# anoma/taiga

Measured on NVIDIA H100. Metric: partial-tx proofs/sec, higher is better.
Workload: dtype u32x8 (255-bit Montgomery integers, Pasta Fp/Fq)

## Files before the change

### taiga_b200/csrc/msm_batch.cu

```cuda
#define TB_NOINLINE_MUL 0
#include <cuda.h>
#include <algorithm>
#include <memory>
#include <type_traits>
#include "common.cuh"
#include "kernels.cuh"

namespace tb {

constexpr int BA_THREADS = 256;
constexpr int BA_M = 32;
constexpr int BA_BWD_MINB = 3;
constexpr int BA_MAX_NB = 4096;
constexpr int SORT_THREADS = 1024;
constexpr int SORT_TILE = 1024;
constexpr int SORT_BOX = 256;

__device__ __forceinline__ void block_scan_excl(uint32_t* v, int n, uint32_t* tmp) {
  const int T = blockDim.x, t = threadIdx.x, per = (n + T - 1) / T;
  const int b0 = t * per, b1 = min(n, b0 + per);
  uint32_t local = 0;
  for (int i = b0; i < b1; ++i) local += v[i];
  uint32_t incl = local;
  const int lane = t & 31, warp = t >> 5, nw = (T + 31) >> 5;
#pragma unroll
  for (int d = 1; d < 32; d <<= 1) { uint32_t o = __shfl_up_sync(0xffffffffu, incl, d); if (lane >= d) incl += o; }
  if (lane == 31) tmp[warp] = incl;
  __syncthreads();
  if (warp == 0) {
    uint32_t w = lane < nw ? tmp[lane] : 0u, wi = w;
#pragma unroll
    for (int d = 1; d < 32; d <<= 1) { uint32_t o = __shfl_up_sync(0xffffffffu, wi, d); if (lane >= d) wi += o; }
    if (lane < nw) tmp[lane] = wi - w;
    if (lane == nw - 1) v[n] = wi;
  }
  __syncthreads();
  uint32_t run = tmp[warp] + incl - local;
  for (int i = b0; i < b1; ++i) { uint32_t x = v[i]; v[i] = run; run += x; }
  __syncthreads();
}

__device__ __forceinline__ uint32_t smem_u32(const void* p) { return (uint32_t)__cvta_generic_to_shared(p); }
__device__ __forceinline__ void mbar_init(uint64_t* bar, uint32_t count) {
  asm volatile("mbarrier.init.shared::cta.b64 [%0], %1;" ::"r"(smem_u32(bar)), "r"(count) : "memory");
}
__device__ __forceinline__ void mbar_expect_tx(uint64_t* bar, uint32_t bytes) {
  asm volatile("mbarrier.arrive.expect_tx.shared::cta.b64 _, [%0], %1;" ::"r"(smem_u32(bar)), "r"(bytes) : "memory");
}
__device__ __forceinline__ void mbar_wait(uint64_t* bar, uint32_t parity) {
  uint32_t done = 0;
  for (uint32_t spin = 0; spin < (1u << 26); ++spin) {
    asm volatile("{ .reg .pred p; mbarrier.try_wait.parity.shared::cta.b64 p, [%1], %2; selp.u32 %0, 1, 0, p; }" : "=r"(done) : "r"(smem_u32(bar)), "r"(parity) : "memory");
    if (done) return;
  }
  __trap();
}
__device__ __forceinline__ void tma_load_tile(void* dst, const CUtensorMap* map, uint64_t* bar, int scalar0, int item) {
  asm volatile("cp.async.bulk.tensor.3d.shared::cluster.global.tile.mbarrier::complete_tx::bytes [%0], [%1, {%3, %4, %5}], [%2];"
               ::"r"(smem_u32(dst)), "l"(map), "r"(smem_u32(bar)), "r"(0), "r"(scalar0), "r"(item) : "memory");
}

template <class S, int CT>
__global__ void __launch_bounds__(SORT_THREADS) msm_sort_kernel(const __grid_constant__ CUtensorMap smap, const S* __restrict__ extras, int N, int n_extra, int c_rt, int W_rt,
                                                                 int NB, int table_stride, uint32_t* __restrict__ counts, uint32_t* __restrict__ entries, long long cap0,
                                                                 unsigned long long* __restrict__ total_entries) {
  const int c = CT ? CT : c_rt, W = CT ? (256 + CT - 1) / CT : W_rt;
  extern __shared__ __align__(128) uint8_t sort_smem[];
  S* tile = reinterpret_cast<S*>(sort_smem);
  uint64_t* bars = reinterpret_cast<uint64_t*>(sort_smem + 2 * SORT_TILE * sizeof(S));
  uint32_t* hist = reinterpret_cast<uint32_t*>(bars + 2);
  uint32_t* tmp = hist + NB + 1;
  const int k = blockIdx.x, t = threadIdx.x;
  const uint32_t half = 1u << (c - 1);
  const int ntiles = (N + SORT_TILE - 1) / SORT_TILE;
  if (t == 0) { mbar_init(&bars[0], 1); mbar_init(&bars[1], 1); asm volatile("fence.mbarrier_init.release.cluster;" ::: "memory"); }
  for (int b = t; b <= NB; b += SORT_THREADS) hist[b] = 0;
  __syncthreads();
  uint32_t* ent = entries + (long long)k * cap0;

  auto digits = [&](const S& sm, uint32_t idx, auto scatter_c) {
    constexpr bool scatter = decltype(scatter_c)::value;
    S s = sm.from_mont();
    if (s.is_zero()) return;
    uint32_t carry = 0;
#pragma unroll
    for (int w = 0; w < W; ++w) {
      const int bit = w * c, limb = bit >> 5, off = bit & 31;
      uint64_t v64 = s.l[limb];
      if (limb + 1 < 8) v64 |= (uint64_t)s.l[limb + 1] << 32;
      uint32_t v = ((uint32_t)(v64 >> off) & ((1u << c) - 1)) + carry, neg = 0;
      if (v > half) { v = (1u << c) - v; neg = 1; carry = 1; } else carry = 0;
      if (v) {
        if (scatter) { const uint32_t pos = atomicAdd(&hist[v - 1], 1u); ent[pos] = (uint32_t)(w * table_stride + idx) | (neg << 31); }
        else atomicAdd(&hist[v - 1], 1u);
      }
    }
  };
  auto issue = [&](int stage, int it) {
    const int s0 = it * SORT_TILE;
    int nbox = (N - s0 + SORT_BOX - 1) / SORT_BOX; if (nbox > SORT_TILE / SORT_BOX) nbox = SORT_TILE / SORT_BOX;
    mbar_expect_tx(&bars[stage], (uint32_t)(nbox * SORT_BOX * sizeof(S)));
    for (int j = 0; j < nbox; ++j) tma_load_tile(tile + stage * SORT_TILE + j * SORT_BOX, &smap, &bars[stage], s0 + j * SORT_BOX, k);
  };
  uint32_t phase[2] = {0, 0};
  for (int pass = 0; pass < 2; ++pass) {
    if (t == 0) issue(0, 0);
    for (int it = 0; it < ntiles; ++it) {
      const int st = it & 1;
      if (t == 0 && it + 1 < ntiles) issue(st ^ 1, it + 1);
      mbar_wait(&bars[st], phase[st]); phase[st] ^= 1;
      const int i = it * SORT_TILE + t;
      if (i < N) { if (pass) digits(tile[st * SORT_TILE + t], (uint32_t)i, std::true_type()); else digits(tile[st * SORT_TILE + t], (uint32_t)i, std::false_type()); }
      __syncthreads();
    }
    if (t < n_extra) { const S ex = ldg_fe(extras + (long long)k * n_extra + t); if (pass) digits(ex, (uint32_t)(N + t), std::true_type()); else digits(ex, (uint32_t)(N + t), std::false_type()); }
    __syncthreads();
    if (pass == 0) {
      for (int b = t; b < NB; b += SORT_THREADS) counts[(long long)k * NB + b] = hist[b];
      __syncthreads();
      block_scan_excl(hist, NB, tmp);
      if (t == 0) atomicAdd(total_entries, (unsigned long long)hist[NB]);
    }
  }
}

template <class F> __device__ __forceinline__ void sts_fe(uint4* lo, uint4* hi, int idx, const F& v) {
  lo[idx] = make_uint4(v.l[0], v.l[1], v.l[2], v.l[3]); hi[idx] = make_uint4(v.l[4], v.l[5], v.l[6], v.l[7]);
}
template <class F> __device__ __forceinline__ F lds_fe(const uint4* lo, const uint4* hi, int idx) {
  uint4 x = lo[idx], y = hi[idx]; F v;
  v.l[0] = x.x; v.l[1] = x.y; v.l[2] = x.z; v.l[3] = x.w; v.l[4] = y.x; v.l[5] = y.y; v.l[6] = y.z; v.l[7] = y.w; return v;
}

enum { PK_ADD = 0, PK_DBL, PK_COPY1, PK_COPY2, PK_INF };
constexpr int META_KIND_SHIFT = 28;
constexpr uint32_t META_IN0_MASK = (1u << META_KIND_SHIFT) - 1;

struct RoundOffsets {
  uint32_t* off_cur; uint32_t* off_nxt; uint32_t n_next;
  __device__ __forceinline__ void build(uint8_t* smem, const uint32_t* __restrict__ counts0, int NB, int round) {
    off_cur = reinterpret_cast<uint32_t*>(smem); off_nxt = off_cur + (NB + 4);
    uint32_t* tmp = off_nxt + (NB + 4);
    for (int b = threadIdx.x; b < NB; b += blockDim.x) {
      const uint32_t c0 = counts0[b], cr = (c0 + ((1u << round) - 1)) >> round;
      off_cur[b] = cr; off_nxt[b] = (cr + 1) >> 1;
    }
    __syncthreads();
    block_scan_excl(off_cur, NB, tmp);
    block_scan_excl(off_nxt, NB, tmp);
    n_next = off_nxt[NB];
  }
  __device__ __forceinline__ void locate(uint32_t q, int NB, uint32_t& in0, bool& two, int& hint) const {
    int lo = hint;
#pragma unroll 1
    for (int s = 0; s < 6 && off_nxt[lo + 1] <= q; ++s) ++lo;
    if (off_nxt[lo + 1] <= q) {
      int hi = NB;
      while (hi - lo > 1) { const int mid = (lo + hi) >> 1; if (off_nxt[mid] <= q) lo = mid; else hi = mid; }
    }
    hint = lo;
    in0 = off_cur[lo] + 2 * (q - off_nxt[lo]);
    two = in0 + 1 < off_cur[lo + 1];
  }
};
constexpr size_t ba_off_bytes(int NB) { return (size_t)(2 * (NB + 4) + 32) * 4; }

template <class B> struct Planes {
  B* x; long long cap;
  __device__ __forceinline__ B ldx(uint32_t pos) const { return ldg_fe(x + pos); }
  __device__ __forceinline__ Aff<B> ld(uint32_t pos) const { Aff<B> p; p.x = ldg_fe(x + pos); p.y = ldg_fe(x + cap + pos); return p; }
  __device__ __forceinline__ void st(uint32_t pos, const Aff<B>& p) const { st_fe(x + pos, p.x); st_fe(x + cap + pos, p.y); }
};
template <class B> __device__ __forceinline__ Aff<B> table_point(const Aff<B>* table, uint32_t e) {
  Aff<B> p = ldg_aff(table + (e & 0x7fffffffu));
  if (e >> 31) p.y = p.y.neg();
  return p;
}
template <class B> __device__ __forceinline__ int classify_pair(const Aff<B>& p1, const Aff<B>& p2, B& den) {
  if (p2.is_inf()) return PK_COPY1;
  if (p1.is_inf()) return PK_COPY2;
  den = p2.x - p1.x;
  if (!den.is_zero()) return PK_ADD;
  if (p1.y == p2.y && !p1.y.is_zero()) { den = p1.y.dbl(); return PK_DBL; }
  return PK_INF;
}

__global__ void __launch_bounds__(BA_THREADS) msm_ba_count_kernel(const uint32_t* __restrict__ counts0, int NB, int R, uint32_t* __restrict__ n_items) {
  __shared__ uint32_t red[BA_THREADS / 32];
  const int k = blockIdx.x, t = threadIdx.x;
  for (int r = 0; r <= R; ++r) {
    uint32_t s = 0;
    for (int b = t; b < NB; b += BA_THREADS) s += (counts0[(long long)k * NB + b] + ((1u << r) - 1)) >> r;
    for (int d = 16; d >= 1; d >>= 1) s += __shfl_down_sync(0xffffffffu, s, d);
    if ((t & 31) == 0) red[t >> 5] = s;
    __syncthreads();
    if (t == 0) { uint32_t tot = 0; for (int w = 0; w < BA_THREADS / 32; ++w) tot += red[w]; n_items[(long long)k * (R + 1) + r] = tot; }
    __syncthreads();
  }
}

template <class B, bool FIRST>
__global__ void __launch_bounds__(BA_THREADS) msm_ba_fwd_kernel(const uint32_t* __restrict__ counts0, int NB, int round, const uint32_t* __restrict__ entries,
                                                                 const Aff<B>* __restrict__ table, const B* __restrict__ items_in, long long cap_in, long long cap_out,
                                                                 B* __restrict__ pre, B* __restrict__ tree, uint32_t* __restrict__ meta, uint2* __restrict__ eidx,
                                                                 const uint32_t* __restrict__ n_items, int R) {
  extern __shared__ __align__(16) uint8_t ba_smem[];
  const int k = blockIdx.y, t = threadIdx.x;
  const uint32_t Q0 = blockIdx.x * (BA_M * BA_THREADS);
  if (Q0 >= n_items[(long long)k * (R + 1) + round + 1]) return;
  RoundOffsets ro; ro.build(ba_smem, counts0 + (long long)k * NB, NB, round);
  const uint32_t* ent_k = entries + (long long)k * cap_in;
  const Planes<B> in{const_cast<B*>(items_in) + 2 * (long long)k * cap_in, cap_in};
  B* pre_k = pre + 2 * (long long)k * cap_out;
  uint32_t* meta_k = meta + (long long)k * cap_out;
  uint2* eidx_k = eidx + (long long)k * cap_out;
  B acc = B::one();
  int hint = 0;
#pragma unroll 1
  for (int i = 0; i < BA_M; ++i) {
    const uint32_t q = Q0 + (uint32_t)i * BA_THREADS + t;
    if (q >= ro.n_next) break;
    uint32_t in0; bool two; ro.locate(q, NB, in0, two, hint);
    st_fe(pre_k + q, acc);
    int kind = PK_COPY1;
    uint2 e = make_uint2(0, 0);
    if (FIRST) { e.x = __ldg(ent_k + in0); if (two) e.y = __ldg(ent_k + in0 + 1); eidx_k[q] = e; }
    if (two) {
      const B x1 = FIRST ? ldg_fe(&table[e.x & 0x7fffffffu].x) : in.ldx(in0), x2 = FIRST ? ldg_fe(&table[e.y & 0x7fffffffu].x) : in.ldx(in0 + 1);
      B den = x2 - x1;
      kind = PK_ADD;
      if (den.is_zero() || x1.is_zero() || x2.is_zero()) {
        const Aff<B> p1 = FIRST ? table_point(table, e.x) : in.ld(in0), p2 = FIRST ? table_point(table, e.y) : in.ld(in0 + 1);
        kind = classify_pair(p1, p2, den);
      }
      if (kind == PK_ADD || kind == PK_DBL) acc = acc * den;
    }
    meta_k[q] = in0 | (uint32_t)kind << META_KIND_SHIFT;
  }
  __syncthreads();
  B* nd = reinterpret_cast<B*>(ba_smem);
  nd[BA_THREADS + t] = acc;
  __syncthreads();
  for (int w = BA_THREADS >> 1; w >= 1; w >>= 1) {
    if (t < w) nd[w + t] = nd[2 * (w + t)] * nd[2 * (w + t) + 1];
    __syncthreads();
  }
  B* tr = tree + ((long long)k * gridDim.x + blockIdx.x) * (2 * BA_THREADS);
  st_fe(tr + t, t ? nd[t] : B::one()); st_fe(tr + BA_THREADS + t, nd[BA_THREADS + t]);
}

template <class B>
__global__ void msm_ba_inv_kernel(B* __restrict__ tree, uint32_t n_trees) {
  const uint32_t i = blockIdx.x * blockDim.x + threadIdx.x;
  if (i >= n_trees) return;
  B* root = tree + (size_t)i * (2 * BA_THREADS) + 1;
  st_fe(root, ld_fe(root).inv());
}

template <class B, bool FIRST>
__global__ void __launch_bounds__(BA_THREADS, BA_BWD_MINB) msm_ba_bwd_kernel(const Aff<B>* __restrict__ table, const B* __restrict__ items_in, long long cap_in,
                                                                 B* __restrict__ items_out, long long cap_out, const B* __restrict__ tree,
                                                                 const uint32_t* __restrict__ meta, const uint2* __restrict__ eidx, const uint32_t* __restrict__ n_items, int round, int R) {
  extern __shared__ __align__(16) uint8_t ba_smem[];
  const int k = blockIdx.y, t = threadIdx.x;
  const uint32_t Q0 = blockIdx.x * (BA_M * BA_THREADS);
  const uint32_t n_next = n_items[(long long)k * (R + 1) + round + 1];
  if (Q0 >= n_next) return;
  B* nd = reinterpret_cast<B*>(ba_smem);
  { const B* tr = tree + ((long long)k * gridDim.x + blockIdx.x) * (2 * BA_THREADS);
    nd[t] = ld_fe(tr + t); nd[BA_THREADS + t] = ld_fe(tr + BA_THREADS + t); }
  __syncthreads();
  for (int w = 1; w < BA_THREADS; w <<= 1) {
    B child_inv;
    const int node = w + (t >> 1);
    if (t < 2 * w) child_inv = nd[node] * nd[2 * node + ((t & 1) ^ 1)];
    __syncthreads();
    if (t < 2 * w) nd[2 * node + (t & 1)] = child_inv;
    __syncthreads();
  }
  B inv_run = nd[BA_THREADS + t];
  const Planes<B> in{const_cast<B*>(items_in) + 2 * (long long)k * cap_in, cap_in}, out{items_out + 2 * (long long)k * cap_out, cap_out};
  const uint32_t* meta_k = meta + (long long)k * cap_out;
  const uint2* eidx_k = eidx + (long long)k * cap_out;
  const B* pre_k = out.x + cap_out;
  int last = BA_M - 1;
  while (last >= 0 && Q0 + (uint32_t)last * BA_THREADS + t >= n_next) --last;
#pragma unroll 1
  for (int i = last; i >= 0; --i) {
    const uint32_t q = Q0 + (uint32_t)i * BA_THREADS + t;
    const uint32_t mt = __ldg(meta_k + q);
    const uint2 e = FIRST ? __ldg(eidx_k + q) : make_uint2(0, 0);
    const uint32_t in0 = mt & META_IN0_MASK, kind = mt >> META_KIND_SHIFT;
    const Aff<B> p1 = FIRST ? table_point(table, e.x) : in.ld(in0);
    Aff<B> r;
    if (kind <= PK_DBL) {
      Aff<B> p2 = p1;
      B num, den;
      if (kind == PK_ADD) { p2 = FIRST ? table_point(table, e.y) : in.ld(in0 + 1); num = p2.y - p1.y; den = p2.x - p1.x; }
      else { const B x2 = p1.x.sqr(); num = x2.dbl() + x2; den = p1.y.dbl(); }
      const B dinv = inv_run * ld_fe(pre_k + q);
      inv_run = inv_run * den;
      const B lam = num * dinv;
      r.x = lam.sqr() - p1.x - p2.x;
      r.y = lam * (p1.x - r.x) - p1.y;
    } else {
      r = p1;
      if (kind == PK_COPY2) r = FIRST ? table_point(table, e.y) : in.ld(in0 + 1);
      else if (kind == PK_INF) r = Aff<B>::inf();
    }
    out.st(q, r);
  }
}

template <class B>
__global__ void __launch_bounds__(BA_THREADS) msm_ba_finish_kernel(const uint32_t* __restrict__ counts0, int NB, int round, const B* __restrict__ items, long long cap,
                                                                    Xyzz<B>* __restrict__ buckets) {
  extern __shared__ __align__(16) uint8_t fin_smem[];
  uint32_t* off = reinterpret_cast<uint32_t*>(fin_smem);
  uint32_t* tmp = off + NB + 4;
  const int k = blockIdx.y, t = threadIdx.x;
  for (int b = t; b < NB; b += BA_THREADS) { uint32_t c0 = counts0[(long long)k * NB + b]; off[b] = (c0 + ((1u << round) - 1)) >> round; }
  __syncthreads();
  block_scan_excl(off, NB, tmp);
  const int b = blockIdx.x * BA_THREADS + t;
  if (b >= NB) return;
  Xyzz<B> acc = Xyzz<B>::inf();
  const Planes<B> it{const_cast<B*>(items) + 2 * (long long)k * cap, cap};
  for (uint32_t p = off[b]; p < off[b + 1]; ++p) acc.add_affine(it.ld(p));
  buckets[(long long)k * NB + b] = acc;
}

typedef CUresult (*EncodeTiledFn)(CUtensorMap*, CUtensorMapDataType, cuuint32_t, void*, const cuuint64_t*, const cuuint64_t*, const cuuint32_t*, const cuuint32_t*,
                                  CUtensorMapInterleave, CUtensorMapSwizzle, CUtensorMapL2promotion, CUtensorMapFloatOOBfill);
static EncodeTiledFn encode_tiled_fn() {
  static EncodeTiledFn fn = nullptr;
  if (!fn) {
    void* p = nullptr; cudaDriverEntryPointQueryResult qr;
    TB_CUDA(cudaGetDriverEntryPoint("cuTensorMapEncodeTiled", &p, cudaEnableDefault, &qr));
    if (qr != cudaDriverEntryPointSuccess || !p) throw CudaError("cuTensorMapEncodeTiled is not available from this driver");
    fn = reinterpret_cast<EncodeTiledFn>(p);
  }
  return fn;
}

template <class B, bool FIRST>
static void launch_round(Ctx* ctx, dim3 grid, size_t fwd_smem, size_t bwd_smem, const uint32_t* counts, int NB, int r, const uint32_t* entries, const Aff<B>* table, const B* in,
                         long long cap_in, B* out, long long cap_out, B* pre, B* tree, uint32_t* meta, uint2* eidx, const uint32_t* n_items, int R, uint32_t n_trees) {
  ctx->opt_in_smem(msm_ba_fwd_kernel<B, FIRST>, fwd_smem);
  ctx->opt_in_smem(msm_ba_bwd_kernel<B, FIRST>, bwd_smem);
  launch(ctx, msm_ba_fwd_kernel<B, FIRST>, grid, BA_THREADS, fwd_smem, counts, NB, r, entries, table, in, cap_in, cap_out, pre, tree, meta, eidx, n_items, R);
  launch(ctx, msm_ba_inv_kernel<B>, (n_trees + 63) / 64, 64, 0, tree, n_trees);
  launch(ctx, msm_ba_bwd_kernel<B, FIRST>, grid, BA_THREADS, bwd_smem, table, in, cap_in, out, cap_out, tree, meta, eidx, n_items, r, R);
}

bool msm_batch_applicable(int N, int K, const MsmConfig& cfg, int c) {
  if (cfg.table_windows <= 0 || (1 << (c - 1)) > BA_MAX_NB || c < 6) return false;
  const long long min_terms = tb_tune("TB_MSM_BA_MIN_TERMS", 1 << 21);
  return (long long)N * K >= min_terms;
}

template <class B, class S>
void msm_batch_buckets(Ctx* ctx, const S* scalars, long long sstride, const Aff<B>* table, int N, int K, int c, int W, int table_stride, const S* extras, int n_extra,
                       Xyzz<B>* buckets) {
  const int NB = 1 << (c - 1);
  TB_REQUIRE(((uintptr_t)scalars & 15) == 0 && (sstride * (long long)sizeof(S)) % 16 == 0, "scalar vectors must be 16-byte aligned for TMA");
  const long long cap0 = (long long)(N + n_extra) * W;
  std::vector<long long> cap(1, cap0);
  const int R = tb_tune("TB_MSM_BA_ROUNDS", 10);
  TB_REQUIRE(R >= 1 && R <= 20, "TB_MSM_BA_ROUNDS out of range");
  for (int r = 0; r < R; ++r) cap.push_back((cap.back() + NB + 1) / 2);
  TB_REQUIRE(cap0 <= (long long)META_IN0_MASK + 1, "too many MSM entries for the pair index of meta");
  const int Kc_max = tb_tune("TB_MSM_BA_CHUNK", ctx->sm_count);
  const int Kc = K < Kc_max ? K : Kc_max;
  DevBuf<uint32_t> counts(ctx, (size_t)Kc * NB), entries(ctx, (size_t)Kc * cap0);
  const size_t eidx_fe = ((size_t)Kc * cap[1] + 3) / 4;
  DevBuf<B> itA(ctx, (size_t)Kc * 2 * cap[1]), itB(ctx, std::max(R > 1 ? (size_t)(Kc * 2 * cap[2]) : (size_t)0, eidx_fe));
  uint2* eidx = reinterpret_cast<uint2*>(itB.get());
  const size_t sort_smem = 2 * SORT_TILE * sizeof(S) + 16 + (size_t)(NB + 1 + 32) * 4 + 16;
  const size_t fwd_smem = std::max(ba_off_bytes(NB), (size_t)2 * BA_THREADS * sizeof(B));
  const size_t bwd_smem = (size_t)2 * BA_THREADS * sizeof(B);
  const size_t fin_smem = (size_t)(NB + 4 + 32) * 4;
  ctx->opt_in_smem(msm_sort_kernel<S, 13>, sort_smem);
  ctx->opt_in_smem(msm_sort_kernel<S, 0>, sort_smem);
  ctx->opt_in_smem(msm_ba_finish_kernel<B>, fin_smem);
  const long long pairs_per_cta = (long long)BA_M * BA_THREADS;
  const unsigned ctas1 = (unsigned)((cap[1] + pairs_per_cta - 1) / pairs_per_cta);
  DevBuf<B> tree(ctx, (size_t)Kc * ctas1 * 2 * BA_THREADS);
  DevBuf<uint32_t> meta(ctx, (size_t)Kc * cap[1]), n_items(ctx, (size_t)Kc * (R + 1));
  for (int k0 = 0; k0 < K; k0 += Kc) {
    const int kc = K - k0 < Kc ? K - k0 : Kc;
    { ProfScope ps(ctx, PC_MSM_SORT);
      CUtensorMap smap;
      const cuuint64_t dims[3] = {8, (cuuint64_t)N, (cuuint64_t)kc};
      const cuuint64_t strides[2] = {sizeof(S), (cuuint64_t)sstride * sizeof(S)};
      const cuuint32_t box[3] = {8, SORT_BOX, 1}, estr[3] = {1, 1, 1};
      CUresult cr = encode_tiled_fn()(&smap, CU_TENSOR_MAP_DATA_TYPE_UINT32, 3, const_cast<S*>(scalars + (long long)k0 * sstride), dims, strides, box, estr,
                                      CU_TENSOR_MAP_INTERLEAVE_NONE, CU_TENSOR_MAP_SWIZZLE_NONE, CU_TENSOR_MAP_L2_PROMOTION_L2_128B, CU_TENSOR_MAP_FLOAT_OOB_FILL_NONE);
      if (cr != CUDA_SUCCESS) throw CudaError("cuTensorMapEncodeTiled failed for the scalar tensor (" + std::to_string((int)cr) + ")");
      const S* ex = extras ? extras + (long long)k0 * n_extra : nullptr;
      if (c == 13) launch(ctx, msm_sort_kernel<S, 13>, kc, SORT_THREADS, sort_smem, smap, ex, N, extras ? n_extra : 0, c, W, NB, table_stride, counts.get(), entries.get(), cap0, ctx->d_msm_adds.get());
      else launch(ctx, msm_sort_kernel<S, 0>, kc, SORT_THREADS, sort_smem, smap, ex, N, extras ? n_extra : 0, c, W, NB, table_stride, counts.get(), entries.get(), cap0, ctx->d_msm_adds.get()); }
    { ProfScope ps(ctx, PC_MSM_ACCUM);
      launch(ctx, msm_ba_count_kernel, kc, BA_THREADS, 0, counts.get(), NB, R, n_items.get());
      for (int r = 0; r < R; ++r) {
        const B* in = (r & 1) ? itA.get() : itB.get();
        B* out = (r & 1) ? itB.get() : itA.get();
        const unsigned gx = (unsigned)((cap[r + 1] + pairs_per_cta - 1) / pairs_per_cta);
        dim3 grid(gx, kc);
        const uint32_t n_trees = gx * (uint32_t)kc;
        (r == 0 ? launch_round<B, true> : launch_round<B, false>)(ctx, grid, fwd_smem, bwd_smem, counts.get(), NB, r, entries.get(), table, in, r == 0 ? cap0 : cap[r], out,
                                                                  cap[r + 1], out + cap[r + 1], tree.get(), meta.get(), eidx, n_items.get(), R, n_trees);
      }
      const B* last = (R & 1) ? itA.get() : itB.get();
      launch(ctx, msm_ba_finish_kernel<B>, dim3((NB + BA_THREADS - 1) / BA_THREADS, kc), BA_THREADS, fin_smem, counts.get(), NB, R, last, cap[R], buckets + (size_t)k0 * NB); }
  }
}

template void msm_batch_buckets<Fq, Fp>(Ctx*, const Fp*, long long, const Aff<Fq>*, int, int, int, int, int, const Fp*, int, Xyzz<Fq>*);
template void msm_batch_buckets<Fp, Fq>(Ctx*, const Fq*, long long, const Aff<Fp>*, int, int, int, int, int, const Fq*, int, Xyzz<Fp>*);

}
```

Baseline: 18.34.

## Group batch-affine reduction rounds per thread and fuse next-round forward into backward pass

```diff
diff --git a/taiga_b200/csrc/msm_batch.cu b/taiga_b200/csrc/msm_batch.cu
--- a/taiga_b200/csrc/msm_batch.cu
+++ b/taiga_b200/csrc/msm_batch.cu
@@ -9,8 +9,9 @@
 namespace tb {
 
 constexpr int BA_THREADS = 256;
-constexpr int BA_M = 32;
-constexpr int BA_BWD_MINB = 3;
+constexpr int BA_ITEMS = 64;
+constexpr int BA_GROUP = 4;
+constexpr int BA_BWD_MINB = 2;
 constexpr int BA_MAX_NB = 4096;
 constexpr int SORT_THREADS = 1024;
 constexpr int SORT_TILE = 1024;
@@ -133,42 +134,12 @@
 }
 
 enum { PK_ADD = 0, PK_DBL, PK_COPY1, PK_COPY2, PK_INF };
-constexpr int META_KIND_SHIFT = 28;
-constexpr uint32_t META_IN0_MASK = (1u << META_KIND_SHIFT) - 1;
-
-struct RoundOffsets {
-  uint32_t* off_cur; uint32_t* off_nxt; uint32_t n_next;
-  __device__ __forceinline__ void build(uint8_t* smem, const uint32_t* __restrict__ counts0, int NB, int round) {
-    off_cur = reinterpret_cast<uint32_t*>(smem); off_nxt = off_cur + (NB + 4);
-    uint32_t* tmp = off_nxt + (NB + 4);
-    for (int b = threadIdx.x; b < NB; b += blockDim.x) {
-      const uint32_t c0 = counts0[b], cr = (c0 + ((1u << round) - 1)) >> round;
-      off_cur[b] = cr; off_nxt[b] = (cr + 1) >> 1;
-    }
-    __syncthreads();
-    block_scan_excl(off_cur, NB, tmp);
-    block_scan_excl(off_nxt, NB, tmp);
-    n_next = off_nxt[NB];
-  }
-  __device__ __forceinline__ void locate(uint32_t q, int NB, uint32_t& in0, bool& two, int& hint) const {
-    int lo = hint;
-#pragma unroll 1
-    for (int s = 0; s < 6 && off_nxt[lo + 1] <= q; ++s) ++lo;
-    if (off_nxt[lo + 1] <= q) {
-      int hi = NB;
-      while (hi - lo > 1) { const int mid = (lo + hi) >> 1; if (off_nxt[mid] <= q) lo = mid; else hi = mid; }
-    }
-    hint = lo;
-    in0 = off_cur[lo] + 2 * (q - off_nxt[lo]);
-    two = in0 + 1 < off_cur[lo + 1];
-  }
-};
-constexpr size_t ba_off_bytes(int NB) { return (size_t)(2 * (NB + 4) + 32) * 4; }
 
 template <class B> struct Planes {
   B* x; long long cap;
   __device__ __forceinline__ B ldx(uint32_t pos) const { return ldg_fe(x + pos); }
   __device__ __forceinline__ Aff<B> ld(uint32_t pos) const { Aff<B> p; p.x = ldg_fe(x + pos); p.y = ldg_fe(x + cap + pos); return p; }
+  __device__ __forceinline__ Aff<B> ld_own(uint32_t pos) const { Aff<B> p; p.x = ld_fe(x + pos); p.y = ld_fe(x + cap + pos); return p; }
   __device__ __forceinline__ void st(uint32_t pos, const Aff<B>& p) const { st_fe(x + pos, p.x); st_fe(x + cap + pos, p.y); }
 };
 template <class B> __device__ __forceinline__ Aff<B> table_point(const Aff<B>* table, uint32_t e) {
@@ -185,57 +156,78 @@
   return PK_INF;
 }
 
-__global__ void __launch_bounds__(BA_THREADS) msm_ba_count_kernel(const uint32_t* __restrict__ counts0, int NB, int R, uint32_t* __restrict__ n_items) {
-  __shared__ uint32_t red[BA_THREADS / 32];
+__global__ void __launch_bounds__(BA_THREADS) msm_ba_count_kernel(const uint32_t* __restrict__ counts0, int NB, int R, int S, uint32_t* __restrict__ offs,
+                                                                   uint32_t* __restrict__ blks) {
+  extern __shared__ __align__(16) uint32_t cnt_smem[];
+  uint32_t* v = cnt_smem; uint32_t* tmp = v + NB + 1;
   const int k = blockIdx.x, t = threadIdx.x;
   for (int r = 0; r <= R; ++r) {
-    uint32_t s = 0;
-    for (int b = t; b < NB; b += BA_THREADS) s += (counts0[(long long)k * NB + b] + ((1u << r) - 1)) >> r;
-    for (int d = 16; d >= 1; d >>= 1) s += __shfl_down_sync(0xffffffffu, s, d);
-    if ((t & 31) == 0) red[t >> 5] = s;
-    __syncthreads();
-    if (t == 0) { uint32_t tot = 0; for (int w = 0; w < BA_THREADS / 32; ++w) tot += red[w]; n_items[(long long)k * (R + 1) + r] = tot; }
-    __syncthreads();
-  }
-}
+    for (int pass = 0; pass < (r < R ? 2 : 1); ++pass) {
+      const int g = min(S, R - r);
+      for (int b = t; b < NB; b += BA_THREADS) {
+        const uint32_t a = (counts0[(long long)k * NB + b] + ((1u << r) - 1)) >> r;
+        v[b] = pass ? (a + ((1u << g) - 1)) >> g : a;
+      }
+      __syncthreads();
+      block_scan_excl(v, NB, tmp);
+      uint32_t* dst = pass ? blks + ((long long)k * R + r) * (NB + 1) : offs + ((long long)k * (R + 1) + r) * (NB + 1);
+      for (int b = t; b <= NB; b += BA_THREADS) dst[b] = v[b];
+      __syncthreads();
+    }
+  }
+}
+
 
 template <class B, bool FIRST>
-__global__ void __launch_bounds__(BA_THREADS) msm_ba_fwd_kernel(const uint32_t* __restrict__ counts0, int NB, int round, const uint32_t* __restrict__ entries,
-                                                                 const Aff<B>* __restrict__ table, const B* __restrict__ items_in, long long cap_in, long long cap_out,
-                                                                 B* __restrict__ pre, B* __restrict__ tree, uint32_t* __restrict__ meta, uint2* __restrict__ eidx,
-                                                                 const uint32_t* __restrict__ n_items, int R) {
+__global__ void __launch_bounds__(BA_THREADS, 3) msm_ba_fwd_kernel(const uint32_t* __restrict__ offs, const uint32_t* __restrict__ blks, int NB, int round, int g, int R,
+                                                                 const uint32_t* __restrict__ entries, const Aff<B>* __restrict__ table, const B* __restrict__ items_in,
+                                                                 long long cap_in, B* __restrict__ items_out, long long cap_out, B* __restrict__ tree,
+                                                                 uint8_t* __restrict__ kind, uint2* __restrict__ eidx, uint2* __restrict__ desc, long long cap_desc, long long cap_slot) {
   extern __shared__ __align__(16) uint8_t ba_smem[];
-  const int k = blockIdx.y, t = threadIdx.x;
-  const uint32_t Q0 = blockIdx.x * (BA_M * BA_THREADS);
-  if (Q0 >= n_items[(long long)k * (R + 1) + round + 1]) return;
-  RoundOffsets ro; ro.build(ba_smem, counts0 + (long long)k * NB, NB, round);
+  const int k = blockIdx.y, t = threadIdx.x, nblk = BA_ITEMS >> g;
+  const uint32_t* blk_g = blks + ((long long)k * R + round) * (NB + 1);
+  const uint32_t n_blk = blk_g[NB], id0 = blockIdx.x * (BA_THREADS * nblk);
+  if (id0 >= n_blk) return;
+  uint32_t* bo = reinterpret_cast<uint32_t*>(ba_smem);
+  for (int b = t; b <= NB; b += BA_THREADS) bo[b] = blk_g[b];
+  __syncthreads();
+  const uint32_t* off_r = offs + ((long long)k * (R + 1) + round) * (NB + 1);
+  const uint32_t* off_n = off_r + (NB + 1);
   const uint32_t* ent_k = entries + (long long)k * cap_in;
   const Planes<B> in{const_cast<B*>(items_in) + 2 * (long long)k * cap_in, cap_in};
-  B* pre_k = pre + 2 * (long long)k * cap_out;
-  uint32_t* meta_k = meta + (long long)k * cap_out;
-  uint2* eidx_k = eidx + (long long)k * cap_out;
+  B* pre_k = items_out + (2 * (long long)k + 1) * cap_out;
+  const long long side = (long long)k * cap_slot + (long long)blockIdx.x * (BA_THREADS * (BA_ITEMS / 2)) + t;
+  uint8_t* kind_k = kind + side;
+  uint2* eidx_k = eidx + side;
   B acc = B::one();
-  int hint = 0;
 #pragma unroll 1
-  for (int i = 0; i < BA_M; ++i) {
-    const uint32_t q = Q0 + (uint32_t)i * BA_THREADS + t;
-    if (q >= ro.n_next) break;
-    uint32_t in0; bool two; ro.locate(q, NB, in0, two, hint);
-    st_fe(pre_k + q, acc);
-    int kind = PK_COPY1;
-    uint2 e = make_uint2(0, 0);
-    if (FIRST) { e.x = __ldg(ent_k + in0); if (two) e.y = __ldg(ent_k + in0 + 1); eidx_k[q] = e; }
-    if (two) {
-      const B x1 = FIRST ? ldg_fe(&table[e.x & 0x7fffffffu].x) : in.ldx(in0), x2 = FIRST ? ldg_fe(&table[e.y & 0x7fffffffu].x) : in.ldx(in0 + 1);
-      B den = x2 - x1;
-      kind = PK_ADD;
-      if (den.is_zero() || x1.is_zero() || x2.is_zero()) {
-        const Aff<B> p1 = FIRST ? table_point(table, e.x) : in.ld(in0), p2 = FIRST ? table_point(table, e.y) : in.ld(in0 + 1);
-        kind = classify_pair(p1, p2, den);
+  for (int j = 0; j < nblk; ++j) {
+    const uint32_t id = id0 + (uint32_t)j * BA_THREADS + t;
+    if (id >= n_blk) break;
+    int lo = 0, hi = NB;
+    while (hi - lo > 1) { const int mid = (lo + hi) >> 1; if (bo[mid] <= id) lo = mid; else hi = mid; }
+    const uint32_t jb = id - bo[lo], base = off_r[lo] + (jb << g), q0 = off_n[lo] + (jb << (g - 1));
+    const uint32_t n0 = min(1u << g, off_r[lo + 1] - base);
+    desc[(long long)k * cap_desc + id] = make_uint2((uint32_t)lo | n0 << 16, jb);
+#pragma unroll 1
+    for (uint32_t o = 0; 2 * o < n0; ++o) {
+      const uint32_t in0 = base + 2 * o, q = q0 + o, slot = (((uint32_t)j << (g - 1)) + o) * BA_THREADS;
+      const bool two = 2 * o + 1 < n0;
+      int kd = PK_COPY1;
+      uint2 e = make_uint2(0, 0);
+      if (FIRST) { e.x = __ldg(ent_k + in0); if (two) e.y = __ldg(ent_k + in0 + 1); eidx_k[slot] = e; }
+      if (two) {
+        const B x1 = FIRST ? ldg_fe(&table[e.x & 0x7fffffffu].x) : in.ldx(in0), x2 = FIRST ? ldg_fe(&table[e.y & 0x7fffffffu].x) : in.ldx(in0 + 1);
+        B den = x2 - x1;
+        kd = PK_ADD;
+        if (den.is_zero() || x1.is_zero() || x2.is_zero()) {
+          const Aff<B> p1 = FIRST ? table_point(table, e.x) : in.ld(in0), p2 = FIRST ? table_point(table, e.y) : in.ld(in0 + 1);
+          kd = classify_pair(p1, p2, den);
+        }
+        if (kd <= PK_DBL) { st_fe(pre_k + q, acc); acc = acc * den; }
       }
-      if (kind == PK_ADD || kind == PK_DBL) acc = acc * den;
-    }
-    meta_k[q] = in0 | (uint32_t)kind << META_KIND_SHIFT;
+      kind_k[slot] = (uint8_t)kd;
+    }
   }
   __syncthreads();
   B* nd = reinterpret_cast<B*>(ba_smem);
@@ -257,18 +249,19 @@
   st_fe(root, ld_fe(root).inv());
 }
 
-template <class B, bool FIRST>
-__global__ void __launch_bounds__(BA_THREADS, BA_BWD_MINB) msm_ba_bwd_kernel(const Aff<B>* __restrict__ table, const B* __restrict__ items_in, long long cap_in,
-                                                                 B* __restrict__ items_out, long long cap_out, const B* __restrict__ tree,
-                                                                 const uint32_t* __restrict__ meta, const uint2* __restrict__ eidx, const uint32_t* __restrict__ n_items, int round, int R) {
+template <class B, bool FIRST, bool FUSE>
+__global__ void __launch_bounds__(BA_THREADS, BA_BWD_MINB) msm_ba_bwd_kernel(const uint32_t* __restrict__ offs, const uint32_t* __restrict__ blks, int NB, int g0, int g, int d, int R,
+                                                                 const Aff<B>* __restrict__ table, const B* __restrict__ items_in, long long cap_in,
+                                                                 B* __restrict__ items_out, long long cap_out, B* __restrict__ items_nxt, long long cap_nxt,
+                                                                 B* __restrict__ tree, const uint8_t* __restrict__ kind_in, uint8_t* __restrict__ kind_out,
+                                                                 const uint2* __restrict__ eidx, const uint2* __restrict__ desc, long long cap_desc, long long cap_slot) {
   extern __shared__ __align__(16) uint8_t ba_smem[];
-  const int k = blockIdx.y, t = threadIdx.x;
-  const uint32_t Q0 = blockIdx.x * (BA_M * BA_THREADS);
-  const uint32_t n_next = n_items[(long long)k * (R + 1) + round + 1];
-  if (Q0 >= n_next) return;
+  const int k = blockIdx.y, t = threadIdx.x, nblk = BA_ITEMS >> g;
+  const uint32_t n_blk = blks[((long long)k * R + g0) * (NB + 1) + NB], id0 = blockIdx.x * (BA_THREADS * nblk);
+  if (id0 >= n_blk) return;
   B* nd = reinterpret_cast<B*>(ba_smem);
-  { const B* tr = tree + ((long long)k * gridDim.x + blockIdx.x) * (2 * BA_THREADS);
-    nd[t] = ld_fe(tr + t); nd[BA_THREADS + t] = ld_fe(tr + BA_THREADS + t); }
+  B* tr = tree + ((long long)k * gridDim.x + blockIdx.x) * (2 * BA_THREADS);
+  nd[t] = ld_fe(tr + t); nd[BA_THREADS + t] = ld_fe(tr + BA_THREADS + t);
   __syncthreads();
   for (int w = 1; w < BA_THREADS; w <<= 1) {
     B child_inv;
@@ -279,36 +272,74 @@
     __syncthreads();
   }
   B inv_run = nd[BA_THREADS + t];
+  const int r = g0 + d;
+  const uint32_t* off_r = offs + ((long long)k * (R + 1) + r) * (NB + 1);
   const Planes<B> in{const_cast<B*>(items_in) + 2 * (long long)k * cap_in, cap_in}, out{items_out + 2 * (long long)k * cap_out, cap_out};
-  const uint32_t* meta_k = meta + (long long)k * cap_out;
-  const uint2* eidx_k = eidx + (long long)k * cap_out;
+  const Planes<B> nxt{FUSE ? items_nxt + 2 * (long long)k * cap_nxt : nullptr, cap_nxt};
+  const long long side = (long long)k * cap_slot + t;
+  const uint8_t* kind_k = kind_in + side + (long long)blockIdx.x * (BA_THREADS * (BA_ITEMS >> (d + 1)));
+  uint8_t* kind_n = FUSE ? kind_out + side + (long long)blockIdx.x * (BA_THREADS * (BA_ITEMS >> (d + 2))) : nullptr;
+  const uint2* eidx_k = eidx + side + (long long)blockIdx.x * (BA_THREADS * (BA_ITEMS / 2));
+  const uint2* desc_k = desc + (long long)k * cap_desc;
   const B* pre_k = out.x + cap_out;
-  int last = BA_M - 1;
-  while (last >= 0 && Q0 + (uint32_t)last * BA_THREADS + t >= n_next) --last;
+  const bool rev = !(d & 1);
+  B acc = B::one(), xs;
 #pragma unroll 1
-  for (int i = last; i >= 0; --i) {
-    const uint32_t q = Q0 + (uint32_t)i * BA_THREADS + t;
-    const uint32_t mt = __ldg(meta_k + q);
-    const uint2 e = FIRST ? __ldg(eidx_k + q) : make_uint2(0, 0);
-    const uint32_t in0 = mt & META_IN0_MASK, kind = mt >> META_KIND_SHIFT;
-    const Aff<B> p1 = FIRST ? table_point(table, e.x) : in.ld(in0);
-    Aff<B> r;
-    if (kind <= PK_DBL) {
-      Aff<B> p2 = p1;
-      B num, den;
-      if (kind == PK_ADD) { p2 = FIRST ? table_point(table, e.y) : in.ld(in0 + 1); num = p2.y - p1.y; den = p2.x - p1.x; }
-      else { const B x2 = p1.x.sqr(); num = x2.dbl() + x2; den = p1.y.dbl(); }
-      const B dinv = inv_run * ld_fe(pre_k + q);
-      inv_run = inv_run * den;
-      const B lam = num * dinv;
-      r.x = lam.sqr() - p1.x - p2.x;
-      r.y = lam * (p1.x - r.x) - p1.y;
-    } else {
-      r = p1;
-      if (kind == PK_COPY2) r = FIRST ? table_point(table, e.y) : in.ld(in0 + 1);
-      else if (kind == PK_INF) r = Aff<B>::inf();
-    }
-    out.st(q, r);
+  for (int jj = 0; jj < nblk; ++jj) {
+    const uint32_t id = id0 + (uint32_t)(rev ? nblk - 1 - jj : jj) * BA_THREADS + t;
+    if (id >= n_blk) continue;
+    const uint2 ds = __ldg(desc_k + id);
+    const uint32_t b = ds.x & 0xffffu, n_r = ((ds.x >> 16) + ((1u << d) - 1)) >> d, m = (n_r + 1) >> 1;
+    const uint32_t base = off_r[b] + (ds.y << (g - d)), q0 = off_r[NB + 1 + b] + (ds.y << (g - d - 1));
+    const uint32_t qn0 = FUSE ? off_r[2 * (NB + 1) + b] + (ds.y << (g - d - 2)) : 0;
+    const uint32_t s0 = (uint32_t)(rev ? nblk - 1 - jj : jj) << (g - d - 1);
+#pragma unroll 1
+    for (uint32_t oo = 0; oo < m; ++oo) {
+      const uint32_t o = rev ? m - 1 - oo : oo, q = q0 + o, in0 = base + 2 * o;
+      const uint32_t kind = kind_k[(s0 + o) * BA_THREADS];
+      const uint2 e = FIRST ? __ldg(eidx_k + (s0 + o) * BA_THREADS) : make_uint2(0, 0);
+      const Aff<B> p1 = FIRST ? table_point(table, e.x) : in.ld(in0);
+      Aff<B> res;
+      if (kind <= PK_DBL) {
+        Aff<B> p2 = p1;
+        B num, den;
+        if (kind == PK_ADD) { p2 = FIRST ? table_point(table, e.y) : in.ld(in0 + 1); num = p2.y - p1.y; den = p2.x - p1.x; }
+        else { const B x2 = p1.x.sqr(); num = x2.dbl() + x2; den = p1.y.dbl(); }
+        const B dinv = inv_run * ld_fe(pre_k + q);
+        inv_run = inv_run * den;
+        const B lam = num * dinv;
+        res.x = lam.sqr() - p1.x - p2.x;
+        res.y = lam * (p1.x - res.x) - p1.y;
+      } else {
+        res = p1;
+        if (kind == PK_COPY2) res = FIRST ? table_point(table, e.y) : in.ld(in0 + 1);
+        else if (kind == PK_INF) res = Aff<B>::inf();
+      }
+      out.st(q, res);
+      if (FUSE) {
+        if (rev ? (o & 1) : (!(o & 1) && o + 1 < m)) { xs = res.x; continue; }
+        const uint32_t qn = qn0 + (o >> 1);
+        int kn = PK_COPY1;
+        if ((o | 1) < m) {
+          const B x1 = (o & 1) ? xs : res.x, x2 = (o & 1) ? res.x : xs;
+          B den = x2 - x1;
+          kn = PK_ADD;
+          if (den.is_zero() || x1.is_zero() || x2.is_zero()) kn = classify_pair(out.ld_own(q0 + (o & ~1u)), out.ld_own(q0 + (o | 1)), den);
+          if (kn <= PK_DBL) { st_fe(nxt.x + cap_nxt + qn, acc); acc = acc * den; }
+        }
+        kind_n[((s0 >> 1) + (o >> 1)) * BA_THREADS] = (uint8_t)kn;
+      }
+    }
+  }
+  if (FUSE) {
+    __syncthreads();
+    nd[BA_THREADS + t] = acc;
+    __syncthreads();
+    for (int w = BA_THREADS >> 1; w >= 1; w >>= 1) {
+      if (t < w) nd[w + t] = nd[2 * (w + t)] * nd[2 * (w + t) + 1];
+      __syncthreads();
+    }
+    st_fe(tr + t, t ? nd[t] : B::one()); st_fe(tr + BA_THREADS + t, nd[BA_THREADS + t]);
   }
 }
 
@@ -343,14 +374,33 @@
   return fn;
 }
 
-template <class B, bool FIRST>
-static void launch_round(Ctx* ctx, dim3 grid, size_t fwd_smem, size_t bwd_smem, const uint32_t* counts, int NB, int r, const uint32_t* entries, const Aff<B>* table, const B* in,
-                         long long cap_in, B* out, long long cap_out, B* pre, B* tree, uint32_t* meta, uint2* eidx, const uint32_t* n_items, int R, uint32_t n_trees) {
-  ctx->opt_in_smem(msm_ba_fwd_kernel<B, FIRST>, fwd_smem);
-  ctx->opt_in_smem(msm_ba_bwd_kernel<B, FIRST>, bwd_smem);
-  launch(ctx, msm_ba_fwd_kernel<B, FIRST>, grid, BA_THREADS, fwd_smem, counts, NB, r, entries, table, in, cap_in, cap_out, pre, tree, meta, eidx, n_items, R);
-  launch(ctx, msm_ba_inv_kernel<B>, (n_trees + 63) / 64, 64, 0, tree, n_trees);
-  launch(ctx, msm_ba_bwd_kernel<B, FIRST>, grid, BA_THREADS, bwd_smem, table, in, cap_in, out, cap_out, tree, meta, eidx, n_items, r, R);
+template <class B>
+static void launch_group(Ctx* ctx, int kc, int NB, int R, int g0, int g, const std::vector<long long>& cap, unsigned gx, const uint32_t* offs, const uint32_t* blks,
+                         const uint32_t* entries, const Aff<B>* table, B* const it[3], uint8_t* const kinds[2], B* tree, uint2* eidx, uint2* desc, long long cap_desc, long long cap_slot) {
+  const size_t fwd_smem = std::max((size_t)(NB + 1) * 4, (size_t)2 * BA_THREADS * sizeof(B));
+  const size_t bwd_smem = (size_t)2 * BA_THREADS * sizeof(B);
+  const dim3 grid(gx, kc);
+  const uint32_t n_trees = gx * (uint32_t)kc;
+  auto in_of = [&](int r) { return r == 0 ? (const B*)nullptr : (const B*)it[(r - 1) % 3]; };
+  if (g0 == 0) {
+    ctx->opt_in_smem(msm_ba_fwd_kernel<B, true>, fwd_smem);
+    launch(ctx, msm_ba_fwd_kernel<B, true>, grid, BA_THREADS, fwd_smem, offs, blks, NB, g0, g, R, entries, table, in_of(g0), cap[0], it[0], cap[1], tree, kinds[0], eidx,
+           desc, cap_desc, cap_slot);
+  } else {
+    ctx->opt_in_smem(msm_ba_fwd_kernel<B, false>, fwd_smem);
+    launch(ctx, msm_ba_fwd_kernel<B, false>, grid, BA_THREADS, fwd_smem, offs, blks, NB, g0, g, R, entries, table, in_of(g0), cap[g0], it[g0 % 3], cap[g0 + 1], tree,
+           kinds[g0 % 2], eidx, desc, cap_desc, cap_slot);
+  }
+  for (int d = 0; d < g; ++d) {
+    const int r = g0 + d;
+    const bool fuse = d + 1 < g;
+    auto kern = r == 0 ? (fuse ? msm_ba_bwd_kernel<B, true, true> : msm_ba_bwd_kernel<B, true, false>)
+                       : (fuse ? msm_ba_bwd_kernel<B, false, true> : msm_ba_bwd_kernel<B, false, false>);
+    ctx->opt_in_smem(kern, bwd_smem);
+    launch(ctx, msm_ba_inv_kernel<B>, (n_trees + 63) / 64, 64, 0, tree, n_trees);
+    launch(ctx, kern, grid, BA_THREADS, bwd_smem, offs, blks, NB, g0, g, d, R, table, in_of(r), cap[r], it[r % 3], cap[r + 1], fuse ? it[(r + 1) % 3] : (B*)nullptr,
+           fuse ? cap[r + 2] : 0LL, tree, kinds[r % 2], fuse ? kinds[(r + 1) % 2] : (uint8_t*)nullptr, eidx, desc, cap_desc, cap_slot);
+  }
 }
 
 bool msm_batch_applicable(int N, int K, const MsmConfig& cfg, int c) {
@@ -368,25 +418,42 @@
   std::vector<long long> cap(1, cap0);
   const int R = tb_tune("TB_MSM_BA_ROUNDS", 10);
   TB_REQUIRE(R >= 1 && R <= 20, "TB_MSM_BA_ROUNDS out of range");
+  const int S_grp = tb_tune("TB_MSM_BA_GROUP", BA_GROUP);
+  TB_REQUIRE(S_grp >= 1 && (BA_ITEMS >> S_grp) >= 1, "TB_MSM_BA_GROUP out of range");
   for (int r = 0; r < R; ++r) cap.push_back((cap.back() + NB + 1) / 2);
-  TB_REQUIRE(cap0 <= (long long)META_IN0_MASK + 1, "too many MSM entries for the pair index of meta");
+  TB_REQUIRE(cap0 < (1ll << 32), "too many MSM entries for 32-bit item positions");
   const int Kc_max = tb_tune("TB_MSM_BA_CHUNK", ctx->sm_count);
   const int Kc = K < Kc_max ? K : Kc_max;
   DevBuf<uint32_t> counts(ctx, (size_t)Kc * NB), entries(ctx, (size_t)Kc * cap0);
-  const size_t eidx_fe = ((size_t)Kc * cap[1] + 3) / 4;
-  DevBuf<B> itA(ctx, (size_t)Kc * 2 * cap[1]), itB(ctx, std::max(R > 1 ? (size_t)(Kc * 2 * cap[2]) : (size_t)0, eidx_fe));
-  uint2* eidx = reinterpret_cast<uint2*>(itB.get());
+  struct Group { int g0, g; unsigned gx; };
+  std::vector<Group> groups;
+  long long cap_desc = 0, max_ctas = 0;
+  for (int g0 = 0; g0 < R;) {
+    const int g = std::min(S_grp, R - g0);
+    const long long max_blocks = (cap[g0] + (long long)NB * ((1 << g) - 1)) >> g, per_cta = (long long)BA_THREADS * (BA_ITEMS >> g);
+    const unsigned gx = (unsigned)((max_blocks + per_cta - 1) / per_cta);
+    groups.push_back({g0, g, gx});
+    cap_desc = std::max(cap_desc, (long long)gx * per_cta);
+    max_ctas = std::max(max_ctas, (long long)gx);
+    g0 += g;
+  }
+  const long long cap_slot = max_ctas * BA_THREADS * (BA_ITEMS / 2);
+  const size_t eidx_fe = ((size_t)(Kc * cap_slot) + 3) / 4;
+  DevBuf<B> it0(ctx, (size_t)(Kc * 2 * cap[1])), it1(ctx, R > 1 ? (size_t)(Kc * 2 * cap[2]) : 0), it2(ctx, std::max(R > 2 ? (size_t)(Kc * 2 * cap[3]) : (size_t)0, eidx_fe));
+  B* const it[3] = {it0.get(), it1.get(), it2.get()};
+  uint2* eidx = reinterpret_cast<uint2*>(it2.get());
+  DevBuf<uint8_t> kind0(ctx, (size_t)(Kc * cap_slot)), kind1(ctx, R > 1 ? (size_t)(Kc * cap_slot) : 0);
+  uint8_t* const kinds[2] = {kind0.get(), kind1.get()};
+  DevBuf<B> tree(ctx, (size_t)Kc * max_ctas * 2 * BA_THREADS);
+  DevBuf<uint2> desc(ctx, (size_t)Kc * cap_desc);
+  DevBuf<uint32_t> offs(ctx, (size_t)Kc * (R + 1) * (NB + 1)), blks(ctx, (size_t)Kc * R * (NB + 1));
   const size_t sort_smem = 2 * SORT_TILE * sizeof(S) + 16 + (size_t)(NB + 1 + 32) * 4 + 16;
-  const size_t fwd_smem = std::max(ba_off_bytes(NB), (size_t)2 * BA_THREADS * sizeof(B));
-  const size_t bwd_smem = (size_t)2 * BA_THREADS * sizeof(B);
+  const size_t cnt_smem = (size_t)(NB + 1 + 32) * 4;
   const size_t fin_smem = (size_t)(NB + 4 + 32) * 4;
   ctx->opt_in_smem(msm_sort_kernel<S, 13>, sort_smem);
   ctx->opt_in_smem(msm_sort_kernel<S, 0>, sort_smem);
+  ctx->opt_in_smem(msm_ba_count_kernel, cnt_smem);
   ctx->opt_in_smem(msm_ba_finish_kernel<B>, fin_smem);
-  const long long pairs_per_cta = (long long)BA_M * BA_THREADS;
-  const unsigned ctas1 = (unsigned)((cap[1] + pairs_per_cta - 1) / pairs_per_cta);
-  DevBuf<B> tree(ctx, (size_t)Kc * ctas1 * 2 * BA_THREADS);
-  DevBuf<uint32_t> meta(ctx, (size_t)Kc * cap[1]), n_items(ctx, (size_t)Kc * (R + 1));
   for (int k0 = 0; k0 < K; k0 += Kc) {
     const int kc = K - k0 < Kc ? K - k0 : Kc;
     { ProfScope ps(ctx, PC_MSM_SORT);
@@ -401,18 +468,12 @@
       if (c == 13) launch(ctx, msm_sort_kernel<S, 13>, kc, SORT_THREADS, sort_smem, smap, ex, N, extras ? n_extra : 0, c, W, NB, table_stride, counts.get(), entries.get(), cap0, ctx->d_msm_adds.get());
       else launch(ctx, msm_sort_kernel<S, 0>, kc, SORT_THREADS, sort_smem, smap, ex, N, extras ? n_extra : 0, c, W, NB, table_stride, counts.get(), entries.get(), cap0, ctx->d_msm_adds.get()); }
     { ProfScope ps(ctx, PC_MSM_ACCUM);
-      launch(ctx, msm_ba_count_kernel, kc, BA_THREADS, 0, counts.get(), NB, R, n_items.get());
-      for (int r = 0; r < R; ++r) {
-        const B* in = (r & 1) ? itA.get() : itB.get();
-        B* out = (r & 1) ? itB.get() : itA.get();
-        const unsigned gx = (unsigned)((cap[r + 1] + pairs_per_cta - 1) / pairs_per_cta);
-        dim3 grid(gx, kc);
-        const uint32_t n_trees = gx * (uint32_t)kc;
-        (r == 0 ? launch_round<B, true> : launch_round<B, false>)(ctx, grid, fwd_smem, bwd_smem, counts.get(), NB, r, entries.get(), table, in, r == 0 ? cap0 : cap[r], out,
-                                                                  cap[r + 1], out + cap[r + 1], tree.get(), meta.get(), eidx, n_items.get(), R, n_trees);
-      }
-      const B* last = (R & 1) ? itA.get() : itB.get();
-      launch(ctx, msm_ba_finish_kernel<B>, dim3((NB + BA_THREADS - 1) / BA_THREADS, kc), BA_THREADS, fin_smem, counts.get(), NB, R, last, cap[R], buckets + (size_t)k0 * NB); }
+      launch(ctx, msm_ba_count_kernel, kc, BA_THREADS, cnt_smem, counts.get(), NB, R, S_grp, offs.get(), blks.get());
+      for (const Group& gr : groups)
+        launch_group<B>(ctx, kc, NB, R, gr.g0, gr.g, cap, gr.gx, offs.get(), blks.get(), entries.get(), table, it, kinds, tree.get(), eidx, desc.get(), cap_desc,
+                          cap_slot);
+      launch(ctx, msm_ba_finish_kernel<B>, dim3((NB + BA_THREADS - 1) / BA_THREADS, kc), BA_THREADS, fin_smem, counts.get(), NB, R, it[(R - 1) % 3], cap[R],
+             buckets + (size_t)k0 * NB); }
   }
 }
 
```

Result: slower. 16.37 (median of 6 runs) (-10.7%).
